# kkahatapitiya/Coarse-Fine-Networks

Measured on AMD Instinct MI355X. Metric: clips/sec (fwd+bwd+SGD) x3d_fine X3D-M T=256x224x224, higher is better.
Workload: dtype f32; 1 GPU; x3d_fine X3D-M train step (fwd+loss+bwd+SGD), 8x3x256x224x224 clips per GPU, random-init weights; clips_per_gpu=8, frames=256, parallelism=dp1, launch=eager

## Files before the change

coarse-fine-networks_amd/cfn_hip/ops.py:

```python
import torch
from torch.autograd import Function
from torch.autograd.function import once_differentiable

import ctypes
import os
import threading

from . import call, call_try, check, query, last_error, ACT_NONE, ACT_RELU, ACT_SWISH, ACT_SIGMOID


_scratch_epoch = [0]


class _ZeroArena(object):
    CHUNK = 1 << 20

    def __init__(self):
        self.buf, self.off, self.epoch = {}, {}, _scratch_epoch[0]

    def take(self, numel, dev):
        if self.epoch != _scratch_epoch[0]:
            self.buf, self.off, self.epoch = {}, {}, _scratch_epoch[0]
        numel_al = (numel + 1) & ~1
        key = (dev.type, dev.index)
# ... 440 lines not shown
        if want_w:
            g64, fin = _gw_buffers(ctx.wparam, C, 5, x.device)
        fused = want_x and want_w and call_try('cfn_dwconv_t5_bwd_fused' + _sfx(y), gy, y, gs, gq, w2, x, gx, g64, N, C, T, H * W)
        if not fused:
            if want_x:
                call('cfn_dwconv_t5_bwd_data' + _sfx(y), gy, y, gs, gq, w2, gx, N, C, T, H * W)
            if want_w:
                call('cfn_dwconv_t5_bwd_weight' + _sfx(y), gy, y, gs, gq, x, g64, N, C, T, H * W)
        if want_w:
            gw = fin()
        return gx, gw, None, None


def dwconv_t5(x, w, stats=True, out_dtype=None):
    return _DwConvT5.apply(x, w, stats, out_dtype)


class _StemConv(Function):

    @staticmethod
    def forward(ctx, x, w):
        x = check(x).contiguous()
        N, Ci, T, H, W = x.shape
        Co = w.shape[0]
        Ho, Wo = (H + 2 - 3) // 2 + 1, (W + 2 - 3) // 2 + 1
        y = torch.empty(N, Co, T, Ho, Wo, dtype=torch.float32, device=x.device)
        w2 = w.reshape(Co, Ci * 9).contiguous()
        call('cfn_stem_conv_fwd', x, w2, y, N, Ci, Co, T, H, W)
        ctx.save_for_backward(x)
        ctx.wshape = tuple(w.shape)
        ctx.wparam = w
        return y

    @staticmethod
    @once_differentiable
    def backward(ctx, gy):
        (x,) = ctx.saved_tensors
        N, Ci, T, H, W = x.shape
        Co = ctx.wshape[0]
        gw = None
        if ctx.needs_input_grad[1]:
            g64, fin = _gw_buffers(ctx.wparam, Co, Ci * 9, x.device)
            call('cfn_stem_conv_bwd_weight', gy.contiguous(), x, g64, N, Ci, Co, T, H, W)
            gw = fin()
        return None, gw


def stem_conv(x, w):
    return _StemConv.apply(x, w)


def _stem_pair_switch():
    try:
        return int(os.environ.get('CFN_STEM_PAIR', '3'))
    except ValueError:
        raise RuntimeError('CFN_STEM_PAIR must be an integer (bit 0: forward, bit 1: backward), got %r' % os.environ['CFN_STEM_PAIR'])


class _StemPair(Function):

    @staticmethod
    def forward(ctx, x, w_s, w_t, want_stats, run_frames):
        x = check(x).contiguous()
        if x.dtype != torch.float32:
            raise RuntimeError('stem_pair: fp32 clip expected, got %s' % x.dtype)
        N, Ci, T, H, W = x.shape
        Co = w_s.shape[0]
        Ho, Wo = (H + 2 - 3) // 2 + 1, (W + 2 - 3) // 2 + 1
        xs = torch.empty(N, Co, T, Ho, Wo, dtype=torch.float32, device=x.device)
        y = torch.empty_like(xs)
        s = q = None
        if want_stats:
            s, q = _f64(N, Co, x.device), _f64(N, Co, x.device)
        ws2 = w_s.reshape(Co, Ci * 9).contiguous()
        wt2 = w_t.reshape(Co, 5).contiguous()
        if not (_stem_pair_switch() & 1 and call_try('cfn_stem_pair_fwd', x, ws2, wt2, xs, y, s, q, N, Ci, Co, T, H, W, run_frames)):
            call('cfn_stem_conv_fwd', x, ws2, xs, N, Ci, Co, T, H, W)
            call('cfn_dwconv_t5_fwd', xs, wt2, y, s, q, N, Co, T, Ho * Wo)
        ctx.save_for_backward(x, xs, y, wt2)
        ctx.params = (w_s, w_t)
        ctx.run_frames = run_frames
        if not want_stats:
            return y, None, None
        return y, s, q

    @staticmethod
    @once_differentiable
    def backward(ctx, gy, gs, gq):
        x, xs, y, wt2 = ctx.saved_tensors
        w_s, w_t = ctx.params
        N, Ci, T, H, W = x.shape
        _, Co, _, Ho, Wo = xs.shape
        gy = torch.zeros_like(y) if gy is None else gy.contiguous()
        gs, gq = _opt(gs), _opt(gq)
        want_s, want_t = ctx.needs_input_grad[1], ctx.needs_input_grad[2]
        gws = gwt = None
        if want_s and want_t:
            gs64, fin_s = _gw_buffers(w_s, Co, Ci * 9, x.device)
            gt64, fin_t = _gw_buffers(w_t, Co, 5, x.device)
            if not (_stem_pair_switch() & 2 and
                    call_try('cfn_stem_pair_bwd', gy, y, gs, gq, wt2, xs, x, gt64, gs64, N, Ci, Co, T, H, W, ctx.run_frames)):
                gxs = torch.empty_like(xs)
                if not call_try('cfn_dwconv_t5_bwd_fused', gy, y, gs, gq, wt2, xs, gxs, gt64, N, Co, T, Ho * Wo):
                    call('cfn_dwconv_t5_bwd_data', gy, y, gs, gq, wt2, gxs, N, Co, T, Ho * Wo)
                    call('cfn_dwconv_t5_bwd_weight', gy, y, gs, gq, xs, gt64, N, Co, T, Ho * Wo)
                call('cfn_stem_conv_bwd_weight', gxs, x, gs64, N, Ci, Co, T, H, W)
            gws, gwt = fin_s(), fin_t()
        elif want_t:
            gt64, fin_t = _gw_buffers(w_t, Co, 5, x.device)
            call('cfn_dwconv_t5_bwd_weight', gy, y, gs, gq, xs, gt64, N, Co, T, Ho * Wo)
            gwt = fin_t()
        elif want_s:
            gs64, fin_s = _gw_buffers(w_s, Co, Ci * 9, x.device)
            gxs = torch.empty_like(xs)
            call('cfn_dwconv_t5_bwd_data', gy, y, gs, gq, wt2, gxs, N, Co, T, Ho * Wo)
            call('cfn_stem_conv_bwd_weight', gxs, x, gs64, N, Ci, Co, T, H, W)
            gws = fin_s()
        return None, gws, gwt, None, None


def stem_pair(x, w_s, w_t, stats=True, run_frames=0):
    return _StemPair.apply(x, w_s, w_t, stats, run_frames)


from .u8clips import clip_lut


def _u8_args(frames, lengths, lut):
    if frames.dtype != torch.uint8 or frames.dim() != 5 or frames.shape[4] != 3:
        raise RuntimeError('uint8 frames of shape (N, T, H, W, 3) expected, got %s %s' % (frames.dtype, tuple(frames.shape)))
    if lut.dtype != torch.float32 or lut.numel() != 3 * 256:
        raise RuntimeError('a (3, 256) fp32 table expected (ops.clip_lut), got %s %s' % (lut.dtype, tuple(lut.shape)))
    if lengths is not None:
        if lengths.numel() != frames.shape[0]:
            raise RuntimeError('one length per clip expected: %d clips, lengths %s' % (frames.shape[0], tuple(lengths.shape)))
        lengths = lengths.to(torch.int32).contiguous()
    return frames.contiguous(), lengths, lut.contiguous()


def clip_u8_to_f32(frames, lut, lengths=None):
    frames, lengths, lut = _u8_args(frames, lengths, lut)
    N, T, H, W, _ = frames.shape
    x = torch.empty(N, 3, T, H, W, dtype=torch.float32, device=frames.device)
    call('cfn_clip_u8_to_f32', frames, lut, lengths, x, N, T, H, W)
    return x


class _StemConvU8(Function):

    @staticmethod
    def forward(ctx, frames, lengths, lut, w):
        frames, lengths, lut = _u8_args(frames, lengths, lut)
        N, T, H, W, Ci = frames.shape
        Co = w.shape[0]
        Ho, Wo = (H + 2 - 3) // 2 + 1, (W + 2 - 3) // 2 + 1
        y = torch.empty(N, Co, T, Ho, Wo, dtype=torch.float32, device=frames.device)
        w2 = w.reshape(Co, Ci * 9).contiguous()
        if not call_try('cfn_stem_conv_u8_fwd', frames, lut, lengths, w2, y, N, Ci, Co, T, H, W):
            call('cfn_stem_conv_fwd', clip_u8_to_f32(frames, lut, lengths), w2, y, N, Ci, Co, T, H, W)
        ctx.save_for_backward(frames, lengths, lut)
        ctx.wshape = tuple(w.shape)
        ctx.wparam = w
        return y

    @staticmethod
    @once_differentiable
    def backward(ctx, gy):
# ... 1374 lines not shown
```

coarse-fine-networks_amd/csrc/stempair.hip:

```cpp
#include "cfn_common.h"
#include <stdlib.h>

typedef float __attribute__((ext_vector_type(16))) sp16;
typedef float __attribute__((ext_vector_type(4))) sp4;
typedef float __attribute__((ext_vector_type(2))) sp2;

struct StemPairBwdArgs {
    const float* gy; const float* y; const double* gs; const double* gq; const float* wt; const float* xs; const float* x;
    double* gwt; double* gws;
    int N, T, R, nch, runs, per_block;
};

namespace {
constexpr int SP_WI = 224, SP_WO = 112, SP_RB = 2, SP_RIN = 2 * SP_RB + 1, SP_PITCH = 228;
constexpr int SP_CIS = SP_RIN * SP_PITCH + 24;
constexpr int SP_GP = 2 * SP_WO + 2;
constexpr int SP_P = SP_WI * SP_WI, SP_PO = SP_WO * SP_WO, SP_BANDS = SP_WO / SP_RB, SP_OOB = 0x7fff0000;
constexpr int SP_XU = 3 * SP_RIN * (SP_WI / 4), SP_NXU = (SP_XU + 511) / 512;
constexpr int SP_GU = 24 * SP_RB * (SP_WO / 4), SP_NGU = (SP_GU + 511) / 512;
constexpr int SP_UPC = SP_RB * (SP_WO / 4);

struct SpCur {
    int run, n, band, ta, tb, t;
    __device__ __forceinline__ void start(int r, int R, int nch, int T) {
        run = r;
        band = r % SP_BANDS;
        const int q = r / SP_BANDS, chunk = q % nch;
        n = q / nch;
        ta = chunk * R;
        tb = min(ta + R, T);
        t = ta - 4;
    }
    __device__ __forceinline__ void next(int R, int nch, int T) {
        if (++t == tb) start(run + 1, R, nch, T);
    }
};
}

__device__ __forceinline__ float sp_taps(float a0, float a1, float a2, float a3, float a4, float w0, float w1, float w2, float w3, float w4) {
    return __builtin_fmaf(a4, w4, __builtin_fmaf(a3, w3, __builtin_fmaf(a2, w2, __builtin_fmaf(a0, w0, __fmul_rn(a1, w1)))));
}

template <bool HASY>
__global__ __launch_bounds__(512) void stem_pair_bwd_kernel(const StemPairBwdArgs a) {
    __shared__ __attribute__((aligned(16))) float lds[3 * SP_CIS + 24 * SP_GP];
    float* const img = lds;
    float* const gbuf = lds + 3 * SP_CIS;
    const int tid = threadIdx.x, lane = tid & 63, wave = cfn_uni(tid >> 6), h = lane >> 5, p = lane & 31;
    const int T = a.T, R = a.R, nch = a.nch;

    for (int i = tid; i < 3 * SP_CIS; i += 512) img[i] = 0.0f;

    int xo[SP_NXU], xl[SP_NXU], xr[SP_NXU];
#pragma unroll
    for (int k = 0; k < SP_NXU; ++k) {
        const int e = k * 512 + tid;
        const int rowid = e / (SP_WI / 4), c4 = e - rowid * (SP_WI / 4), ci = rowid / SP_RIN, r = rowid - ci * SP_RIN;
        const bool in = e < SP_XU;
        xo[k] = in ? (int)(((long)ci * T * SP_P + (long)r * SP_WI + c4 * 4) * 4) : SP_OOB;
        xl[k] = in ? ci * SP_CIS + r * SP_PITCH + 4 + c4 * 4 : -1;
        xr[k] = r;
    }
    int go[SP_NGU], gl[SP_NGU], gc[SP_NGU];
    float wk[SP_NGU][5];
#pragma unroll
    for (int k = 0; k < SP_NGU; ++k) {
        const int e = k * 512 + tid;
        const int co = e / SP_UPC, rem = e - co * SP_UPC;
        const bool in = e < SP_GU;
        go[k] = in ? (int)(((long)co * T * SP_PO + rem * 4) * 4) : SP_OOB;
        gl[k] = in ? co * SP_GP + rem * 4 : -1;
        gc[k] = in ? co : 0;
#pragma unroll
        for (int j = 0; j < 5; ++j) wk[k][j] = a.wt[gc[k] * 5 + 4 - j];
    }
    const int ohl = wave >> 2, ow0 = (wave & 3) * 28;
    const int colp = p < 27 ? p : 0;
    const int ci = colp / 9, kh = (colp - ci * 9) / 3, kw = colp - ci * 9 - kh * 3;
    const float* bp = img + ci * SP_CIS + (2 * ohl + kh) * SP_PITCH + 2 * ow0 + kw + 3 + 2 * h;
    const float* ap = gbuf + min(p, 23) * SP_GP + ohl * SP_WO + ow0 + h;

    sp16 acc0, acc1;
#pragma unroll
    for (int r = 0; r < 16; ++r) acc0[r] = acc1[r] = 0.0f;
    float acct[SP_NGU][5];
#pragma unroll
    for (int k = 0; k < SP_NGU; ++k)
#pragma unroll
        for (int j = 0; j < 5; ++j) acct[k][j] = 0.0f;

    const int first = (int)cfn_xcd_remap(blockIdx.x, gridDim.x) * a.per_block, last = min(first + a.per_block, a.runs);
    const unsigned gbytes = (unsigned)((long)24 * T * SP_PO * 4), xbytes = (unsigned)((long)3 * T * SP_P * 4);
    sp4 fg[SP_NGU], fy[SP_NGU], fs[SP_NGU], fx[SP_NXU];
    auto fetch = [&](const SpCur& c) {
        const bool on = c.run < last;
        const int n = on ? c.n : 0, f = c.t + 2;
        const bool fv = on && f >= 0 && f < T, xv = on && c.t >= c.ta;
        __amdgpu_buffer_rsrc_t rg = cfn_rsrc(a.gy + (long)n * 24 * T * SP_PO, gbytes);
        __amdgpu_buffer_rsrc_t ry = cfn_rsrc((HASY ? a.y : a.gy) + (long)n * 24 * T * SP_PO, gbytes);
        __amdgpu_buffer_rsrc_t rs = cfn_rsrc(a.xs + (long)n * 24 * T * SP_PO, gbytes);
        __amdgpu_buffer_rsrc_t rx = cfn_rsrc(a.x + (long)n * 3 * T * SP_P, xbytes);
        const int ih0 = 2 * c.band * SP_RB - 1;
        const int sg = cfn_uni(fv ? (f * SP_PO + c.band * SP_RB * SP_WO) * 4 : 0);
        const int ss = cfn_uni(xv ? (c.t * SP_PO + c.band * SP_RB * SP_WO) * 4 : 0);
        const int sx = cfn_uni(xv ? c.t * SP_P * 4 : 0), rowoff = cfn_uni(ih0 * SP_WI * 4);
#pragma unroll
        for (int k = 0; k < SP_NGU; ++k) {
            fg[k] = __builtin_bit_cast(sp4, __builtin_amdgcn_raw_buffer_load_b128(rg, fv ? go[k] : SP_OOB, sg, 0));
            if (HASY) fy[k] = __builtin_bit_cast(sp4, __builtin_amdgcn_raw_buffer_load_b128(ry, fv ? go[k] : SP_OOB, sg, 0));
        }
#pragma unroll
        for (int k = 0; k < SP_NGU; ++k)
            fs[k] = __builtin_bit_cast(sp4, __builtin_amdgcn_raw_buffer_load_b128(rs, xv ? go[k] : SP_OOB, ss, 0));
#pragma unroll
        for (int k = 0; k < SP_NXU; ++k)
            fx[k] = __builtin_bit_cast(sp4, __builtin_amdgcn_raw_buffer_load_b128(rx, (xv && xo[k] != SP_OOB && ih0 + xr[k] >= 0) ? xo[k] + rowoff : SP_OOB, sx, 0));
    };

    const sp4 zero = {0.f, 0.f, 0.f, 0.f};
    sp4 W[5][SP_NGU];
#pragma unroll
    for (int i = 0; i < 5; ++i)
#pragma unroll
        for (int k = 0; k < SP_NGU; ++k) W[i][k] = zero;
    float gsv[SP_NGU], gqv[SP_NGU];
#pragma unroll
    for (int k = 0; k < SP_NGU; ++k) gsv[k] = gqv[k] = 0.0f;

    SpCur cc, fc;
    cc.start(first, R, nch, T);
    fc = cc;
    __syncthreads();
    fetch(fc);
    fc.next(R, nch, T);
    while (cc.run < last) {
        if (cc.t == cc.ta - 4) {
#pragma unroll
            for (int k = 0; k < SP_NGU; ++k) {
                gsv[k] = a.gs ? (float)a.gs[cc.n * 24 + gc[k]] : 0.0f;
                gqv[k] = (HASY && a.gq) ? 2.0f * (float)a.gq[cc.n * 24 + gc[k]] : 0.0f;
            }
        }
        const bool mm = cc.t >= cc.ta;
        const float m = (cc.t + 2 >= 0 && cc.t + 2 < T) ? 1.0f : 0.0f;
#pragma unroll
        for (int k = 0; k < SP_NGU; ++k) {
            sp4 v = fg[k] + gsv[k];
            if (HASY) v = __builtin_elementwise_fma(fy[k], (sp4){gqv[k], gqv[k], gqv[k], gqv[k]}, v);
            W[4][k] = v * m;
        }
        if (mm) {
#pragma unroll
            for (int k = 0; k < SP_NGU; ++k) {
                sp4 gx;
#pragma unroll
                for (int i = 0; i < 4; ++i)
                    gx[i] = sp_taps(W[0][k][i], W[1][k][i], W[2][k][i], W[3][k][i], W[4][k][i], wk[k][0], wk[k][1], wk[k][2], wk[k][3], wk[k][4]);
                if (gl[k] >= 0) {
                    *reinterpret_cast<sp2*>(gbuf + gl[k]) = (sp2){gx.x, gx.y};
                    *reinterpret_cast<sp2*>(gbuf + gl[k] + 2) = (sp2){gx.z, gx.w};
                }
#pragma unroll
                for (int j = 0; j < 5; ++j) {
                    const sp4 pr = fs[k] * W[4 - j][k];
                    acct[k][j] += (pr.x + pr.y) + (pr.z + pr.w);
                }
            }
#pragma unroll
            for (int k = 0; k < SP_NXU; ++k)
                if (xl[k] >= 0) *reinterpret_cast<sp4*>(img + xl[k]) = fx[k];
            __syncthreads();
        }
        fetch(fc);
        fc.next(R, nch, T);
        if (mm) {
#pragma unroll
            for (int j = 0; j < 14; j += 2) {
                acc0 = __builtin_amdgcn_mfma_f32_32x32x2f32(ap[2 * j], bp[4 * j], acc0, 0, 0, 0);
                acc1 = __builtin_amdgcn_mfma_f32_32x32x2f32(ap[2 * j + 2], bp[4 * j + 4], acc1, 0, 0, 0);
            }
            __syncthreads();
        }
#pragma unroll
        for (int i = 0; i < 4; ++i)
#pragma unroll
            for (int k = 0; k < SP_NGU; ++k) W[i][k] = W[i + 1][k];
        cc.next(R, nch, T);
    }

    __syncthreads();
#pragma unroll
    for (int k = 0; k < SP_NGU; ++k)
        if (gl[k] >= 0) {
#pragma unroll
            for (int j = 0; j < 5; ++j) lds[(k * 512 + tid) * 5 + j] = acct[k][j];
        }
    __syncthreads();
    if (tid < 24 * 5) {
        const int co = tid / 5, j = tid - co * 5;
        float s = 0.0f;
        for (int u = 0; u < SP_UPC; ++u) s += lds[(co * SP_UPC + u) * 5 + j];
        cfn_add64(&a.gwt[co * 5 + j], (double)s);
    }
    __syncthreads();
#pragma unroll
    for (int r = 0; r < 16; ++r) lds[(wave * 16 + r) * 64 + lane] = acc0[r] + acc1[r];
    __syncthreads();
    for (int e = tid; e < 16 * 64; e += 512) {
        const int r = e >> 6, l = e & 63, hh = l >> 5, col = l & 31;
        const int co = (r & 3) + 8 * (r >> 2) + 4 * hh;
        float s = 0.0f;
#pragma unroll
        for (int w = 0; w < 8; ++w) s += lds[(w * 16 + r) * 64 + l];
        if (co < 24 && col < 27) cfn_add64(&a.gws[co * 27 + col], (double)s);
    }
}

static int stem_pair_plan(int N, int T, int wgs) {
    int best = T;
    long best_cost = -1;
    for (int nch = 1; nch == 1 || T / nch >= 32; ++nch) {
        const int R = cfn_cdiv(T, nch);
        const long runs = (long)N * cfn_cdiv(T, R) * SP_BANDS, per = (runs + wgs - 1) / wgs, cost = per * (R + 2);
        if (best_cost < 0 || cost < best_cost) { best_cost = cost; best = R; }
    }
    return best;
}

static int stem_pair_cus() {
    static int cus = 0;
    if (!cus) { int dev = 0; hipDeviceProp_t pr; cus = (hipGetDevice(&dev) == hipSuccess && hipGetDeviceProperties(&pr, dev) == hipSuccess) ? pr.multiProcessorCount : 256; }
    return cus;
}

static bool stem_pair_shape_ok(int Cimg, int Cout, int T, int Hi, int Wi) {
    return Cimg == 3 && Cout == 24 && Hi == SP_WI && Wi == SP_WI && (long)24 * T * SP_PO * 4 < 0x7fff0000L;
}

extern "C" int cfn_stem_pair_bwd(const float* gy, const float* y, const double* gsum, const double* gsumsq, const float* w_t, const float* xs,
                                 const float* x, double* gw_t, double* gw_s, int N, int Cimg, int Cout, int T, int Hi, int Wi, int run_frames,
                                 void* stream) {
    CFN_REQUIRE(gy && w_t && xs && x && gw_t && gw_s, "cfn_stem_pair_bwd: null tensor");
    CFN_REQUIRE(gsumsq == nullptr || y != nullptr, "cfn_stem_pair_bwd: gsumsq needs y");
    CFN_REQUIRE(N > 0 && Cimg > 0 && Cout > 0 && T > 0 && Hi > 0 && Wi > 0 && run_frames >= 0, "cfn_stem_pair_bwd: bad shape");
    if (!stem_pair_shape_ok(Cimg, Cout, T, Hi, Wi)) return -1;
    const bool hasy = y != nullptr && gsumsq != nullptr;
    if ((((uintptr_t)gy | (uintptr_t)xs | (uintptr_t)x | (uintptr_t)(hasy ? y : gy)) & 15) != 0) return -1;
    const int wgs = stem_pair_cus();
    const int R = run_frames > 0 ? (run_frames < T ? run_frames : T) : stem_pair_plan(N, T, wgs);
    const int nch = cfn_cdiv(T, R);
    const long runs = (long)N * nch * SP_BANDS;
    if (runs >= (1L << 30)) return -1;
    long blocks = runs < wgs ? runs : wgs;
    const long per = (runs + blocks - 1) / blocks;
    blocks = (runs + per - 1) / per;
    StemPairBwdArgs a = {gy, hasy ? y : nullptr, gsum, hasy ? gsumsq : nullptr, w_t, xs, x, gw_t, gw_s, N, T, R, nch, (int)runs, (int)per};
    hipStream_t st = (hipStream_t)stream;
    CfnProfScope prof(CFN_K_STEM, st, 4.0 * N * T * ((double)3 * SP_P + (double)24 * SP_PO * (hasy ? 3 : 2)));
    if (hasy) hipLaunchKernelGGL(stem_pair_bwd_kernel<true>, dim3((unsigned)blocks), dim3(512), 0, st, a);
    else hipLaunchKernelGGL(stem_pair_bwd_kernel<false>, dim3((unsigned)blocks), dim3(512), 0, st, a);
    return cfn_check_launch("stem_pair_bwd");
}

static constexpr __host__ __device__ int sp_tap(int k) { return k < 27 ? (k / 9) * SP_CIS + ((k % 9) / 3) * SP_PITCH + k % 3 : 0; }

struct StemPairFwdArgs {
    const float* x; const float* ws; const float* wt; float* xs; float* y; double* s1; double* s2;
    int N, T, R, nch, runs;
};

__global__ __launch_bounds__(448, 4) void stem_pair_fwd_kernel(const StemPairFwdArgs a) {
    constexpr int NT = 448, NXU = (SP_XU + NT - 1) / NT, KP = 14;
    __shared__ __attribute__((aligned(16))) float img[2][3 * SP_CIS];
    __shared__ __attribute__((aligned(16))) float wts[24 * 8];
    __shared__ float wsl[14 * 64];
    __shared__ float red[2][7][24];
    const int tid = threadIdx.x, lane = tid & 63, wave = cfn_uni(tid >> 6), half = lane >> 5, col = lane & 31;
    const int T = a.T;
    SpCur c;
    c.start((int)cfn_xcd_remap(blockIdx.x, gridDim.x), a.R, a.nch, T);
    const int n = c.n, band = c.band, ta = c.ta, tb = c.tb;

    for (int i = tid; i < 2 * 3 * SP_CIS; i += NT) (&img[0][0])[i] = 0.0f;
    if (tid < 24 * 5) wts[(tid / 5) * 8 + tid % 5] = a.wt[tid];

    const int ih0 = 2 * band * SP_RB - 1;
    int xo[NXU], xl[NXU];
#pragma unroll
    for (int k = 0; k < NXU; ++k) {
        const int e = k * NT + tid;
        const int rowid = e / (SP_WI / 4), c4 = e - rowid * (SP_WI / 4), ci = rowid / SP_RIN, r = rowid - ci * SP_RIN;
        const bool in = e < SP_XU;
        xo[k] = (in && ih0 + r >= 0) ? (int)(((long)ci * T * SP_P + (long)(ih0 + r) * SP_WI + c4 * 4) * 4) : SP_OOB;
        xl[k] = in ? ci * SP_CIS + r * SP_PITCH + 4 + c4 * 4 : -1;
    }
    if (wave == 0) {
#pragma unroll
        for (int s = 0; s < KP; ++s) {
            const int k = 2 * s + half;
            wsl[s * 64 + lane] = (k < 27 && col < 24) ? a.ws[col * 27 + k] : 0.0f;
        }
    }
    const int pos = wave * 32 + col, ohl = pos / SP_WO, ow = pos - ohl * SP_WO;
    const int lboff = 2 * ohl * SP_PITCH + 2 * ow + 3;

    const unsigned gbytes = (unsigned)((long)24 * T * SP_PO * 4), xbytes = (unsigned)((long)3 * T * SP_P * 4);
    __amdgpu_buffer_rsrc_t rx = cfn_rsrc(a.x + (long)n * 3 * T * SP_P, xbytes);
    __amdgpu_buffer_rsrc_t rs = cfn_rsrc(a.xs + (long)n * 24 * T * SP_PO, gbytes);
    __amdgpu_buffer_rsrc_t ry = cfn_rsrc(a.y + (long)n * 24 * T * SP_PO, gbytes);
    const int vout = (half * 4 * T * SP_PO + band * SP_RB * SP_WO + pos) * 4;

    sp4 fx[NXU];
    auto fetch = [&](int s) {
        const bool fv = s >= 0 && s < T && s <= tb + 1;
        const int sx = cfn_uni(fv ? s * SP_P * 4 : 0);
#pragma unroll
        for (int k = 0; k < NXU; ++k)
            fx[k] = __builtin_bit_cast(sp4, __builtin_amdgcn_raw_buffer_load_b128(rx, fv ? xo[k] : SP_OOB, sx, 0));
    };
    auto put = [&](int b) {
#pragma unroll
        for (int k = 0; k < NXU; ++k)
            if (xl[k] >= 0) *reinterpret_cast<sp4*>(&img[b][xl[k]]) = fx[k];
    };

    float W[5][12], st1[12], st2[12];
#pragma unroll
    for (int r = 0; r < 12; ++r) {
        st1[r] = st2[r] = 0.0f;
#pragma unroll
        for (int i = 0; i < 5; ++i) W[i][r] = 0.0f;
    }

    fetch(ta - 2);
    __syncthreads();
    put(0);
    fetch(ta - 1);
    __syncthreads();
    int b = 0;
    for (int s = ta - 2; s <= tb + 1; ++s, b ^= 1) {
        put(b ^ 1);
        fetch(s + 2);
        const float* lb = &img[b][lboff];
        int hsel = half;
        asm volatile("" : "+v"(hsel));
        sp16 acc;
#pragma unroll
        for (int r = 0; r < 16; ++r) acc[r] = 0.0f;
#pragma unroll
        for (int k = 0; k < KP; ++k) acc = __builtin_amdgcn_mfma_f32_32x32x2f32(wsl[k * 64 + lane], lb[hsel ? sp_tap(2 * k + 1) : sp_tap(2 * k)], acc, 0, 0, 0);
        const bool own = s >= ta && s < tb, emit = s - 2 >= ta;
#pragma unroll
        for (int r = 0; r < 12; ++r) {
            const int cr = (r & 3) + 8 * (r >> 2);
            W[4][r] = acc[r];
            __builtin_amdgcn_raw_buffer_store_b32(__builtin_bit_cast(unsigned, W[4][r]), rs, own ? vout : SP_OOB, cfn_uni(own ? (cr * T + s) * SP_PO * 4 : 0), 0);
        }
        if (emit) {
#pragma unroll
            for (int r = 0; r < 12; ++r) {
                const int cr = (r & 3) + 8 * (r >> 2);
                const float* wk = wts + (cr + 4 * half) * 8;
                const float yv = sp_taps(W[0][r], W[1][r], W[2][r], W[3][r], W[4][r], wk[0], wk[1], wk[2], wk[3], wk[4]);
                __builtin_amdgcn_raw_buffer_store_b32(__builtin_bit_cast(unsigned, yv), ry, vout, cfn_uni((cr * T + s - 2) * SP_PO * 4), 0);
                st1[r] += yv;
                st2[r] += yv * yv;
            }
        }
#pragma unroll
        for (int i = 0; i < 4; ++i)
#pragma unroll
            for (int r = 0; r < 12; ++r) W[i][r] = W[i + 1][r];
        __syncthreads();
    }
    if (a.s1) {
#pragma unroll
        for (int r = 0; r < 12; ++r) {
#pragma unroll
            for (int o = 16; o > 0; o >>= 1) { st1[r] += __shfl_xor(st1[r], o, 64); st2[r] += __shfl_xor(st2[r], o, 64); }
            if (col == 0) {
                const int co = (r & 3) + 8 * (r >> 2) + 4 * half;
                red[0][wave][co] = st1[r];
                red[1][wave][co] = st2[r];
            }
        }
        __syncthreads();
        if (tid < 48) {
            const int which = tid / 24, co = tid - which * 24;
            float v = 0.0f;
#pragma unroll
            for (int w = 0; w < 7; ++w) v += red[which][w][co];
            cfn_add64((which ? a.s2 : a.s1) + n * 24 + co, (double)v);
        }
    }
}

static int stem_pair_fwd_plan(int N, int T, int slots) {
    int best = T;
    long best_cost = -1;
    for (int nch = 1; nch == 1 || T / nch >= 32; ++nch) {
        const int R = cfn_cdiv(T, nch);
        const long runs = (long)N * cfn_cdiv(T, R) * SP_BANDS, rounds = (runs + slots - 1) / slots, cost = rounds * (R + 4);
        if (best_cost < 0 || cost < best_cost) { best_cost = cost; best = R; }
    }
    return best;
}

extern "C" int cfn_stem_pair_fwd(const float* x, const float* w_s, const float* w_t, float* xs, float* y, double* sum, double* sumsq, int N,
                                 int Cimg, int Cout, int T, int Hi, int Wi, int run_frames, void* stream) {
    CFN_REQUIRE(x && w_s && w_t && xs && y, "cfn_stem_pair_fwd: null tensor");
    CFN_REQUIRE((sum == nullptr) == (sumsq == nullptr), "cfn_stem_pair_fwd: sum/sumsq mismatch");
    CFN_REQUIRE(N > 0 && Cimg > 0 && Cout > 0 && T > 0 && Hi > 0 && Wi > 0 && run_frames >= 0, "cfn_stem_pair_fwd: bad shape");
    if (!stem_pair_shape_ok(Cimg, Cout, T, Hi, Wi)) return -1;
    if ((((uintptr_t)x | (uintptr_t)xs | (uintptr_t)y) & 15) != 0) return -1;
    const int R = run_frames > 0 ? (run_frames < T ? run_frames : T) : stem_pair_fwd_plan(N, T, 2 * stem_pair_cus());
    const int nch = cfn_cdiv(T, R);
    const long runs = (long)N * nch * SP_BANDS;
    if (runs >= (1L << 30)) return -1;
    StemPairFwdArgs a = {x, w_s, w_t, xs, y, sum, sumsq, N, T, R, nch, (int)runs};
    hipStream_t st = (hipStream_t)stream;
    CfnProfScope prof(CFN_K_STEM, st, 4.0 * N * T * ((double)3 * SP_P + (double)24 * SP_PO * 2));
    hipLaunchKernelGGL(stem_pair_fwd_kernel, dim3((unsigned)runs), dim3(448), 0, st, a);
    return cfn_check_launch("stem_pair_fwd");
}
```

include/cfn_hip.h:

```cpp
#ifndef CFN_HIP_H
#define CFN_HIP_H
#ifdef __cplusplus
extern "C" {
#endif

const char* cfn_last_error(void);
const char* cfn_version(void);
int cfn_device_info(int* cus, int* lds_per_cu, char* name, int name_len);

int cfn_prof_enable(int family, int on);
int cfn_prof_collect(int family, double* total_ms, long* launches, double* total_bytes);

int cfn_dwconv3d_fwd(const float* x, const double* A, const double* B, int act, const float* w, float* y, double* sum,
                     double* sumsq, int N, int C, int T, int Hi, int Wi, int stride, void* stream);
int cfn_dwconv3d_bwd_data(const float* gy, const float* y, const double* gsum, const double* gsumsq, const float* w,
                          const float* x, const double* A, const double* B, int act, float* gx, double* gA, double* gB,
                          int N, int C, int T, int Hi, int Wi, int stride, void* stream);
int cfn_dwconv3d_bwd_weight(const float* gy, const float* y, const double* gsum, const double* gsumsq, const float* x,
                            const double* A, const double* B, int act, double* gw, int N, int C, int T, int Hi, int Wi,
                            int stride, void* stream);
int cfn_dwconv3d_bwd_fused(const float* gy, const float* y, const double* gsum, const double* gsumsq, const float* w,
                           const float* x, const double* A, const double* B, int act, float* gx, double* gA, double* gB,
                           double* gw, int N, int C, int T, int H, int W, void* stream);
int cfn_dwconv3d_bwd_fused_s2(const float* gy, const float* y, const double* gsum, const double* gsumsq, const float* w,
                              const float* x, const double* A, const double* B, int act, float* gx, double* gA, double* gB,
                              double* gw, int N, int C, int T, int H, int W, void* stream);

int cfn_dwconv_t5_fwd(const float* x, const float* w, float* y, double* sum, double* sumsq, int N, int C, int T,
                      long plane, void* stream);
int cfn_dwconv_t5_bwd_data(const float* gy, const float* y, const double* gsum, const double* gsumsq, const float* w,
                           float* gx, int N, int C, int T, long plane, void* stream);
int cfn_dwconv_t5_bwd_weight(const float* gy, const float* y, const double* gsum, const double* gsumsq, const float* x,
                             double* gw, int N, int C, int T, long plane, void* stream);
int cfn_dwconv_t5_bwd_fused(const float* gy, const float* y, const double* gsum, const double* gsumsq, const float* w,
                            const float* x, float* gx, double* gw, int N, int C, int T, long plane, void* stream);

int cfn_pwconv_fwd(const float* x, const double* A, const double* B, int act, const float* w, float* y, double* sum,
                   double* sumsq, int N, int Cin, int Cout, int T, int Hi, int Wi, int stride, void* stream);
int cfn_pwconv_bwd_data(const float* gy, const float* y, const double* gsum, const double* gsumsq, const float* w,
                        const float* x, const double* A, const double* B, int act, float* gx, double* gA, double* gB, int N,
                        int Cin, int Cout, int T, int Hi, int Wi, int stride, void* stream);
int cfn_pwconv_bwd_data_acc(const float* gy, const float* y, const double* gsum, const double* gsumsq, const float* w,
                        const float* x, const double* A, const double* B, int act, float* gx, double* gA, double* gB, int N,
                        int Cin, int Cout, int T, int Hi, int Wi, int stride, const float* acc, int acc_stride,
                        const double* gscale, void* stream);
int cfn_pwconv_bwd_weight(const float* gy, const float* y, const double* gsum, const double* gsumsq, const float* x,
                          const double* A, const double* B, int act, double* gw, int N, int Cin, int Cout, int T, int Hi,
                          int Wi, int stride, const double* gscale, void* stream);

int cfn_pw_split_terms(int terms);

int cfn_pwconv_route(int op, int N, int Cin, int Cout, int T, int Hi, int Wi, int stride, int act, int flags, char* out, int cap);

int cfn_deterministic(int on);

int cfn_pwconv_bwd_fused(const float* gy, const float* y, const double* gsum, const double* gsumsq, const float* w,
                         const float* x, const double* A, const double* B, int act, float* gx, double* gA, double* gB,
                         double* gw, int N, int Cin, int Cout, int T, int Hi, int Wi, const float* acc, int acc_stride,
                         const double* gscale, void* stream);

int cfn_pwconv_short_bwd(const float* gy, const float* y, const double* gsum, const double* gsumsq, const double* gscale,
                         const float* w, const float* x, const double* A, const double* B, int act, float* da, double* gw,
                         int N, int Cin, int Cout, int T, int Hi, int Wi, int stride, void* stream);

int cfn_stem_conv_fwd(const float* x, const float* w, float* y, int N, int Cimg, int Cout, int T, int Hi, int Wi,
                      void* stream);
int cfn_stem_conv_bwd_weight(const float* gy, const float* x, double* gw, int N, int Cimg, int Cout, int T, int Hi, int Wi,
                             void* stream);

int cfn_stem_pair_fwd(const float* x, const float* w_s, const float* w_t, float* xs, float* y, double* sum, double* sumsq, int N,
                      int Cimg, int Cout, int T, int Hi, int Wi, int run_frames, void* stream);
int cfn_stem_pair_bwd(const float* gy, const float* y, const double* gsum, const double* gsumsq, const float* w_t, const float* xs,
                      const float* x, double* gw_t, double* gw_s, int N, int Cimg, int Cout, int T, int Hi, int Wi, int run_frames,
                      void* stream);

int cfn_clip_u8_to_f32(const unsigned char* frames, const float* lut, const int* lengths, float* x, int N, int T, int H, int W,
                       void* stream);
int cfn_stem_conv_u8_fwd(const unsigned char* frames, const float* lut, const int* lengths, const float* w, float* y, int N,
                         int Cimg, int Cout, int T, int Hi, int Wi, void* stream);
int cfn_stem_conv_u8_bwd_weight(const float* gy, const unsigned char* frames, const float* lut, const int* lengths, double* gw,
                                int N, int Cimg, int Cout, int T, int Hi, int Wi, void* stream);

int cfn_bn_fold_fwd(const double* s, const double* q, const float* gamma, const float* beta, float* run_mean, float* run_var,
                    long* nbt, int training, int N, int C, int S, double count, double eps, double momentum, const float* w1,
                    const float* b1, const float* w2, const float* b2, int Wd, double pool_count, double* A, double* B,
                    double* mean, double* rstd, float* A0, float* B0, float* gate, float* hbuf, float* pooled, void* stream);
int cfn_bn_fold_bwd(const double* gA, const double* gB, const double* s, const float* gamma, const double* mean,
                    const double* rstd, const float* A0, const float* B0, const float* gate, const float* hbuf,
                    const float* pooled, const float* w1, const float* w2, int training, int N, int C, int S, int Wd,
                    double count, double pool_count, double* gs, double* gq, float* ggamma, float* gbeta, float* gw1,
                    float* gb1, float* gw2, float* gb2, double* tA, double* tB, void* stream);

int cfn_conv3d_dense_fwd(const float* x, const double* A, const double* B, int act, const float* w, float* y, double* sum,
                         double* sumsq, int N, int Cin, int Cout, int T, int Hi, int Wi, const int* geom, void* stream);
int cfn_conv3d_dense_bwd_data(const float* gy, const float* y, const double* gsum, const double* gsumsq, const float* w,
                              const float* x, const double* A, const double* B, int act, float* gx, double* gA, double* gB,
                              int N, int Cin, int Cout, int T, int Hi, int Wi, const int* geom, void* stream);
int cfn_conv3d_dense_bwd_weight(const float* gy, const float* y, const double* gsum, const double* gsumsq, const float* x,
                                const double* A, const double* B, int act, double* gw, int N, int Cin, int Cout, int T, int Hi,
                                int Wi, const int* geom, void* stream);
int cfn_conv3d_dense_route(int op, int N, int Cin, int Cout, int T, int Hi, int Wi, const int* geom, int flags, int cus, char* out, int cap);

int cfn_gauss_align_fwd(const long* meta, const float* mask, const float* gx, double tx, double ratio, float* GX, int B, int crops,
                        int Tf, int K, void* stream);
int cfn_gauss_align_bwd(const float* gGX, const long* meta, const float* mask, const float* gx, double tx, double ratio,
                        float* ggx, int B, int crops, int Tf, int K, void* stream);

int cfn_fusion_gather_fwd(const float* x, const float* at_raw, const float* at_bias, const float* GX, const float* mask, float* z,
                          float* den, int B, int crops, int C, int Tf, int K, int P, void* stream);
int cfn_fusion_gather_bwd(const float* gz, const float* z, const float* den, const float* x, const float* at_raw,
                          const float* at_bias, const float* GX, const float* mask, float* gx, float* gat, float* gGX, float* dw,
                          int B, int crops, int C, int Tf, int K, int P, void* stream);

int cfn_bn_add_relu_fwd(const float* y, const double* A, const double* B, const float* res, const double* Ar, const double* Br,
                        float* out, int* mask, long NC, long vol, void* stream);
int cfn_bn_add_relu_bwd(const float* gout, const float* gout2, const float* out, const float* y, const double* A, const float* res,
                        const double* Ar, float* gy, float* gres, double* gA, double* gB, double* gAr, long NC, long vol,
                        void* stream);
long cfn_bn_add_relu_mask_words(long NC, long vol);
int cfn_bn_add_relu_bwd_g(const float* gout, const float* gout2, const float* out, const int* mask, const float* y,
                          const float* res, float* g, double* gA, double* gB, double* gAr, long NC, long vol, void* stream);

int cfn_affine_act_fwd(const float* x, const double* A, const double* B, int act, float* out, long NC, long vol, void* stream);
int cfn_affine_act_bwd(const float* gout, const float* x, const double* A, const double* B, int act, float* gx, double* gA,
                       double* gB, long NC, long vol, void* stream);
int cfn_channel_stats(const float* x, double* sum, double* sumsq, long NC, long vol, void* stream);

// ... 222 lines not shown
```

Measured before the change: 107.7 clips/s.

## Recompute stem conv output in backward instead of storing intermediate xs

The forward stem pair kernel gains a variant that skips writing the intermediate spatial conv output xs. The backward kernel gains an RC variant that recomputes xs per tile in LDS from the already-staged input image using MFMA with the spatial weights, then uses it for the temporal weight gradient. This removes a full activation-sized write in forward and a read in backward, and saves memory. The cost is extra MFMA work and LDS in the backward kernel, which could lower occupancy.

After: 108.3 clips/s (median of 6 runs). No clear change (+0.6%).

```diff
diff --git a/coarse-fine-networks_amd/cfn_hip/ops.py b/coarse-fine-networks_amd/cfn_hip/ops.py
--- a/coarse-fine-networks_amd/cfn_hip/ops.py
+++ b/coarse-fine-networks_amd/cfn_hip/ops.py
@@ -516,9 +516,15 @@
 
 def _stem_pair_switch():
     try:
-        return int(os.environ.get('CFN_STEM_PAIR', '3'))
+        return int(os.environ.get('CFN_STEM_PAIR', '7'))
     except ValueError:
-        raise RuntimeError('CFN_STEM_PAIR must be an integer (bit 0: forward, bit 1: backward), got %r' % os.environ['CFN_STEM_PAIR'])
+        raise RuntimeError('CFN_STEM_PAIR must be an integer (bit 0: forward, bit 1: backward, bit 2: do not keep xs), got %r'
+                           % os.environ['CFN_STEM_PAIR'])
+
+
+def _stem_pair_rc_accepts(x, y, Ci, Co, run_frames):
+    N, _, T, H, W = x.shape
+    return query('cfn_stem_pair_bwd_rc_accepts', y.data_ptr(), y.data_ptr(), x.data_ptr(), N, Ci, Co, T, H, W, run_frames) == 1
 
 
 class _StemPair(Function):
@@ -531,17 +537,25 @@
         N, Ci, T, H, W = x.shape
         Co = w_s.shape[0]
         Ho, Wo = (H + 2 - 3) // 2 + 1, (W + 2 - 3) // 2 + 1
-        xs = torch.empty(N, Co, T, Ho, Wo, dtype=torch.float32, device=x.device)
-        y = torch.empty_like(xs)
+        y = torch.empty(N, Co, T, Ho, Wo, dtype=torch.float32, device=x.device)
         s = q = None
         if want_stats:
             s, q = _f64(N, Co, x.device), _f64(N, Co, x.device)
         ws2 = w_s.reshape(Co, Ci * 9).contiguous()
         wt2 = w_t.reshape(Co, 5).contiguous()
-        if not (_stem_pair_switch() & 1 and call_try('cfn_stem_pair_fwd', x, ws2, wt2, xs, y, s, q, N, Ci, Co, T, H, W, run_frames)):
-            call('cfn_stem_conv_fwd', x, ws2, xs, N, Ci, Co, T, H, W)
-            call('cfn_dwconv_t5_fwd', xs, wt2, y, s, q, N, Co, T, Ho * Wo)
-        ctx.save_for_backward(x, xs, y, wt2)
+        sw = _stem_pair_switch()
+        xs = None
+        if not ((sw & 7) == 7 and _stem_pair_rc_accepts(x, y, Ci, Co, run_frames)
+                and call_try('cfn_stem_pair_fwd', x, ws2, wt2, None, y, s, q, N, Ci, Co, T, H, W, run_frames)):
+            xs = torch.empty_like(y)
+            if not (sw & 1 and call_try('cfn_stem_pair_fwd', x, ws2, wt2, xs, y, s, q, N, Ci, Co, T, H, W, run_frames)):
+                call('cfn_stem_conv_fwd', x, ws2, xs, N, Ci, Co, T, H, W)
+                call('cfn_dwconv_t5_fwd', xs, wt2, y, s, q, N, Co, T, Ho * Wo)
+        if xs is None:
+            ctx.save_for_backward(x, y, wt2, ws2)
+        else:
+            ctx.save_for_backward(x, y, wt2, xs)
+        ctx.kept_xs = xs is not None
         ctx.params = (w_s, w_t)
         ctx.run_frames = run_frames
         if not want_stats:
@@ -551,32 +565,44 @@
     @staticmethod
     @once_differentiable
     def backward(ctx, gy, gs, gq):
-        x, xs, y, wt2 = ctx.saved_tensors
+        x, y, wt2, last = ctx.saved_tensors
         w_s, w_t = ctx.params
         N, Ci, T, H, W = x.shape
-        _, Co, _, Ho, Wo = xs.shape
+        _, Co, _, Ho, Wo = y.shape
         gy = torch.zeros_like(y) if gy is None else gy.contiguous()
         gs, gq = _opt(gs), _opt(gq)
         want_s, want_t = ctx.needs_input_grad[1], ctx.needs_input_grad[2]
         gws = gwt = None
+        kept = ctx.kept_xs
+
+        def stored_xs():
+            if kept:
+                return last
+            xs = torch.empty_like(y)
+            call('cfn_stem_conv_fwd', x, last, xs, N, Ci, Co, T, H, W)
+            return xs
+
         if want_s and want_t:
             gs64, fin_s = _gw_buffers(w_s, Co, Ci * 9, x.device)
             gt64, fin_t = _gw_buffers(w_t, Co, 5, x.device)
-            if not (_stem_pair_switch() & 2 and
-                    call_try('cfn_stem_pair_bwd', gy, y, gs, gq, wt2, xs, x, gt64, gs64, N, Ci, Co, T, H, W, ctx.run_frames)):
-                gxs = torch.empty_like(xs)
-                if not call_try('cfn_dwconv_t5_bwd_fused', gy, y, gs, gq, wt2, xs, gxs, gt64, N, Co, T, Ho * Wo):
-                    call('cfn_dwconv_t5_bwd_data', gy, y, gs, gq, wt2, gxs, N, Co, T, Ho * Wo)
-                    call('cfn_dwconv_t5_bwd_weight', gy, y, gs, gq, xs, gt64, N, Co, T, Ho * Wo)
-                call('cfn_stem_conv_bwd_weight', gxs, x, gs64, N, Ci, Co, T, H, W)
+            sw = _stem_pair_switch()
+            if not ((sw & 6) == 6 and not kept and
+                    call_try('cfn_stem_pair_bwd_rc', gy, y, gs, gq, wt2, last, x, gt64, gs64, N, Ci, Co, T, H, W, ctx.run_frames)):
+                xs = stored_xs()
+                if not (sw & 2 and call_try('cfn_stem_pair_bwd', gy, y, gs, gq, wt2, xs, x, gt64, gs64, N, Ci, Co, T, H, W, ctx.run_frames)):
+                    gxs = torch.empty_like(xs)
+                    if not call_try('cfn_dwconv_t5_bwd_fused', gy, y, gs, gq, wt2, xs, gxs, gt64, N, Co, T, Ho * Wo):
+                        call('cfn_dwconv_t5_bwd_data', gy, y, gs, gq, wt2, gxs, N, Co, T, Ho * Wo)
+                        call('cfn_dwconv_t5_bwd_weight', gy, y, gs, gq, xs, gt64, N, Co, T, Ho * Wo)
+                    call('cfn_stem_conv_bwd_weight', gxs, x, gs64, N, Ci, Co, T, H, W)
             gws, gwt = fin_s(), fin_t()
         elif want_t:
             gt64, fin_t = _gw_buffers(w_t, Co, 5, x.device)
-            call('cfn_dwconv_t5_bwd_weight', gy, y, gs, gq, xs, gt64, N, Co, T, Ho * Wo)
+            call('cfn_dwconv_t5_bwd_weight', gy, y, gs, gq, stored_xs(), gt64, N, Co, T, Ho * Wo)
             gwt = fin_t()
         elif want_s:
             gs64, fin_s = _gw_buffers(w_s, Co, Ci * 9, x.device)
-            gxs = torch.empty_like(xs)
+            gxs = torch.empty_like(y)
             call('cfn_dwconv_t5_bwd_data', gy, y, gs, gq, wt2, gxs, N, Co, T, Ho * Wo)
             call('cfn_stem_conv_bwd_weight', gxs, x, gs64, N, Ci, Co, T, H, W)
             gws = fin_s()
diff --git a/coarse-fine-networks_amd/csrc/stempair.hip b/coarse-fine-networks_amd/csrc/stempair.hip
--- a/coarse-fine-networks_amd/csrc/stempair.hip
+++ b/coarse-fine-networks_amd/csrc/stempair.hip
@@ -7,6 +7,7 @@
 
 struct StemPairBwdArgs {
     const float* gy; const float* y; const double* gs; const double* gq; const float* wt; const float* xs; const float* x;
+    const float* ws;
     double* gwt; double* gws;
     int N, T, R, nch, runs, per_block;
 };
@@ -41,15 +42,25 @@
     return __builtin_fmaf(a4, w4, __builtin_fmaf(a3, w3, __builtin_fmaf(a2, w2, __builtin_fmaf(a0, w0, __fmul_rn(a1, w1)))));
 }
 
-template <bool HASY>
+static constexpr __host__ __device__ int sp_tap(int k) { return k < 27 ? (k / 9) * SP_CIS + ((k % 9) / 3) * SP_PITCH + k % 3 : 0; }
+
+template <bool HASY, bool RC>
 __global__ __launch_bounds__(512) void stem_pair_bwd_kernel(const StemPairBwdArgs a) {
-    __shared__ __attribute__((aligned(16))) float lds[3 * SP_CIS + 24 * SP_GP];
+    __shared__ __attribute__((aligned(16))) float lds[3 * SP_CIS + 24 * SP_GP + (RC ? 24 * SP_GP + 14 * 64 : 0)];
     float* const img = lds;
     float* const gbuf = lds + 3 * SP_CIS;
+    float* const xsb = gbuf + 24 * SP_GP;
+    float* const wsl = xsb + 24 * SP_GP;
     const int tid = threadIdx.x, lane = tid & 63, wave = cfn_uni(tid >> 6), h = lane >> 5, p = lane & 31;
     const int T = a.T, R = a.R, nch = a.nch;
 
     for (int i = tid; i < 3 * SP_CIS; i += 512) img[i] = 0.0f;
+    if constexpr (RC) {
+        for (int i = tid; i < 14 * 64; i += 512) {
+            const int k = 2 * (i >> 6) + ((i & 63) >> 5), co = i & 31;
+            wsl[i] = (k < 27 && co < 24) ? a.ws[co * 27 + k] : 0.0f;
+        }
+    }
 
     int xo[SP_NXU], xl[SP_NXU], xr[SP_NXU];
 #pragma unroll
@@ -79,6 +90,9 @@
     const int ci = colp / 9, kh = (colp - ci * 9) / 3, kw = colp - ci * 9 - kh * 3;
     const float* bp = img + ci * SP_CIS + (2 * ohl + kh) * SP_PITCH + 2 * ow0 + kw + 3 + 2 * h;
     const float* ap = gbuf + min(p, 23) * SP_GP + ohl * SP_WO + ow0 + h;
+    const float* xb = img + 2 * ohl * SP_PITCH + 2 * (ow0 + min(p, 27)) + 3;
+    float* const xw = xsb + 4 * h * SP_GP + ohl * SP_WO + ow0 + p;
+    const float* const xb1 = xb + h, * const xb2 = xb + h * (SP_PITCH - 2);
 
     sp16 acc0, acc1;
 #pragma unroll
@@ -98,7 +112,7 @@
         const bool fv = on && f >= 0 && f < T, xv = on && c.t >= c.ta;
         __amdgpu_buffer_rsrc_t rg = cfn_rsrc(a.gy + (long)n * 24 * T * SP_PO, gbytes);
         __amdgpu_buffer_rsrc_t ry = cfn_rsrc((HASY ? a.y : a.gy) + (long)n * 24 * T * SP_PO, gbytes);
-        __amdgpu_buffer_rsrc_t rs = cfn_rsrc(a.xs + (long)n * 24 * T * SP_PO, gbytes);
+        __amdgpu_buffer_rsrc_t rs = cfn_rsrc((RC ? a.gy : a.xs) + (long)n * 24 * T * SP_PO, gbytes);
         __amdgpu_buffer_rsrc_t rx = cfn_rsrc(a.x + (long)n * 3 * T * SP_P, xbytes);
         const int ih0 = 2 * c.band * SP_RB - 1;
         const int sg = cfn_uni(fv ? (f * SP_PO + c.band * SP_RB * SP_WO) * 4 : 0);
@@ -109,9 +123,11 @@
             fg[k] = __builtin_bit_cast(sp4, __builtin_amdgcn_raw_buffer_load_b128(rg, fv ? go[k] : SP_OOB, sg, 0));
             if (HASY) fy[k] = __builtin_bit_cast(sp4, __builtin_amdgcn_raw_buffer_load_b128(ry, fv ? go[k] : SP_OOB, sg, 0));
         }
-#pragma unroll
-        for (int k = 0; k < SP_NGU; ++k)
-            fs[k] = __builtin_bit_cast(sp4, __builtin_amdgcn_raw_buffer_load_b128(rs, xv ? go[k] : SP_OOB, ss, 0));
+        if constexpr (!RC) {
+#pragma unroll
+            for (int k = 0; k < SP_NGU; ++k)
+                fs[k] = __builtin_bit_cast(sp4, __builtin_amdgcn_raw_buffer_load_b128(rs, xv ? go[k] : SP_OOB, ss, 0));
+        }
 #pragma unroll
         for (int k = 0; k < SP_NXU; ++k)
             fx[k] = __builtin_bit_cast(sp4, __builtin_amdgcn_raw_buffer_load_b128(rx, (xv && xo[k] != SP_OOB && ih0 + xr[k] >= 0) ? xo[k] + rowoff : SP_OOB, sx, 0));
@@ -160,10 +176,12 @@
                     *reinterpret_cast<sp2*>(gbuf + gl[k]) = (sp2){gx.x, gx.y};
                     *reinterpret_cast<sp2*>(gbuf + gl[k] + 2) = (sp2){gx.z, gx.w};
                 }
-#pragma unroll
-                for (int j = 0; j < 5; ++j) {
-                    const sp4 pr = fs[k] * W[4 - j][k];
-                    acct[k][j] += (pr.x + pr.y) + (pr.z + pr.w);
+                if constexpr (!RC) {
+#pragma unroll
+                    for (int j = 0; j < 5; ++j) {
+                        const sp4 pr = fs[k] * W[4 - j][k];
+                        acct[k][j] += (pr.x + pr.y) + (pr.z + pr.w);
+                    }
                 }
             }
 #pragma unroll
@@ -174,12 +192,41 @@
         fetch(fc);
         fc.next(R, nch, T);
         if (mm) {
+            if constexpr (RC) {
+                int hsel = h;
+                asm volatile("" : "+v"(hsel));
+                sp16 xa;
+#pragma unroll
+                for (int r = 0; r < 16; ++r) xa[r] = 0.0f;
+#pragma unroll
+                for (int k = 0; k < 14; ++k) {
+                    const int d = sp_tap(2 * k + 1) - sp_tap(2 * k);
+                    const float bv = d == 1 ? xb1[sp_tap(2 * k)] : d == SP_PITCH - 2 ? xb2[sp_tap(2 * k)] : xb[hsel ? sp_tap(2 * k + 1) : sp_tap(2 * k)];
+                    xa = __builtin_amdgcn_mfma_f32_32x32x2f32(wsl[k * 64 + lane], bv, xa, 0, 0, 0);
+                }
+                if (p < 28) {
+#pragma unroll
+                    for (int r = 0; r < 12; ++r) xw[((r & 3) + 8 * (r >> 2)) * SP_GP] = xa[r];
+                }
+            }
 #pragma unroll
             for (int j = 0; j < 14; j += 2) {
                 acc0 = __builtin_amdgcn_mfma_f32_32x32x2f32(ap[2 * j], bp[4 * j], acc0, 0, 0, 0);
                 acc1 = __builtin_amdgcn_mfma_f32_32x32x2f32(ap[2 * j + 2], bp[4 * j + 4], acc1, 0, 0, 0);
             }
             __syncthreads();
+            if constexpr (RC) {
+#pragma unroll
+                for (int k = 0; k < SP_NGU; ++k) {
+                    const float* const xp = xsb + max(gl[k], 0);
+                    const sp2 lo = *reinterpret_cast<const sp2*>(xp), hi = *reinterpret_cast<const sp2*>(xp + 2);
+#pragma unroll
+                    for (int j = 0; j < 5; ++j) {
+                        const sp2 pl = lo * (sp2){W[4 - j][k].x, W[4 - j][k].y}, ph = hi * (sp2){W[4 - j][k].z, W[4 - j][k].w};
+                        acct[k][j] += (pl.x + pl.y) + (ph.x + ph.y);
+                    }
+                }
+            }
         }
 #pragma unroll
         for (int i = 0; i < 4; ++i)
@@ -237,38 +284,72 @@
     return Cimg == 3 && Cout == 24 && Hi == SP_WI && Wi == SP_WI && (long)24 * T * SP_PO * 4 < 0x7fff0000L;
 }
 
+static bool stem_pair_bwd_accepts(const float* gy, const float* y, const float* xs, const float* x, int N, int Cimg, int Cout, int T, int Hi, int Wi,
+                                  int run_frames, int* R_out) {
+    if (N <= 0 || T <= 0 || run_frames < 0 || !stem_pair_shape_ok(Cimg, Cout, T, Hi, Wi)) return false;
+    if ((((uintptr_t)gy | (uintptr_t)xs | (uintptr_t)x | (uintptr_t)y) & 15) != 0) return false;
+    const int R = run_frames > 0 ? (run_frames < T ? run_frames : T) : stem_pair_plan(N, T, stem_pair_cus());
+    if ((long)N * cfn_cdiv(T, R) * SP_BANDS >= (1L << 30)) return false;
+    if (R_out) *R_out = R;
+    return true;
+}
+
+static int stem_pair_bwd_launch(const char* what, const float* gy, const float* y, const double* gsum, const double* gsumsq, const float* w_t,
+                                const float* xs, const float* w_s, const float* x, double* gw_t, double* gw_s, int N, int Cimg, int Cout, int T,
+                                int Hi, int Wi, int run_frames, void* stream) {
+    const bool hasy = y != nullptr && gsumsq != nullptr, rc = xs == nullptr;
+    int R = 0;
+    if (!stem_pair_bwd_accepts(gy, hasy ? y : gy, xs, x, N, Cimg, Cout, T, Hi, Wi, run_frames, &R)) return -1;
+    const int wgs = stem_pair_cus();
+    const int nch = cfn_cdiv(T, R);
+    const long runs = (long)N * nch * SP_BANDS;
+    long blocks = runs < wgs ? runs : wgs;
+    const long per = (runs + blocks - 1) / blocks;
+    blocks = (runs + per - 1) / per;
+    StemPairBwdArgs a = {gy, hasy ? y : nullptr, gsum, hasy ? gsumsq : nullptr, w_t, xs, x, w_s, gw_t, gw_s, N, T, R, nch, (int)runs, (int)per};
+    hipStream_t st = (hipStream_t)stream;
+    CfnProfScope prof(CFN_K_STEM, st, 4.0 * N * T * ((double)3 * SP_P + (double)24 * SP_PO * ((hasy ? 3 : 2) - (rc ? 1 : 0))));
+    const dim3 grid((unsigned)blocks), block(512);
+    if (rc) {
+        if (hasy) hipLaunchKernelGGL((stem_pair_bwd_kernel<true, true>), grid, block, 0, st, a);
+        else hipLaunchKernelGGL((stem_pair_bwd_kernel<false, true>), grid, block, 0, st, a);
+    } else {
+        if (hasy) hipLaunchKernelGGL((stem_pair_bwd_kernel<true, false>), grid, block, 0, st, a);
+        else hipLaunchKernelGGL((stem_pair_bwd_kernel<false, false>), grid, block, 0, st, a);
+    }
+    return cfn_check_launch(what);
+}
+
 extern "C" int cfn_stem_pair_bwd(const float* gy, const float* y, const double* gsum, const double* gsumsq, const float* w_t, const float* xs,
                                  const float* x, double* gw_t, double* gw_s, int N, int Cimg, int Cout, int T, int Hi, int Wi, int run_frames,
                                  void* stream) {
     CFN_REQUIRE(gy && w_t && xs && x && gw_t && gw_s, "cfn_stem_pair_bwd: null tensor");
     CFN_REQUIRE(gsumsq == nullptr || y != nullptr, "cfn_stem_pair_bwd: gsumsq needs y");
     CFN_REQUIRE(N > 0 && Cimg > 0 && Cout > 0 && T > 0 && Hi > 0 && Wi > 0 && run_frames >= 0, "cfn_stem_pair_bwd: bad shape");
-    if (!stem_pair_shape_ok(Cimg, Cout, T, Hi, Wi)) return -1;
-    const bool hasy = y != nullptr && gsumsq != nullptr;
-    if ((((uintptr_t)gy | (uintptr_t)xs | (uintptr_t)x | (uintptr_t)(hasy ? y : gy)) & 15) != 0) return -1;
-    const int wgs = stem_pair_cus();
-    const int R = run_frames > 0 ? (run_frames < T ? run_frames : T) : stem_pair_plan(N, T, wgs);
-    const int nch = cfn_cdiv(T, R);
-    const long runs = (long)N * nch * SP_BANDS;
-    if (runs >= (1L << 30)) return -1;
-    long blocks = runs < wgs ? runs : wgs;
-    const long per = (runs + blocks - 1) / blocks;
-    blocks = (runs + per - 1) / per;
-    StemPairBwdArgs a = {gy, hasy ? y : nullptr, gsum, hasy ? gsumsq : nullptr, w_t, xs, x, gw_t, gw_s, N, T, R, nch, (int)runs, (int)per};
-    hipStream_t st = (hipStream_t)stream;
-    CfnProfScope prof(CFN_K_STEM, st, 4.0 * N * T * ((double)3 * SP_P + (double)24 * SP_PO * (hasy ? 3 : 2)));
-    if (hasy) hipLaunchKernelGGL(stem_pair_bwd_kernel<true>, dim3((unsigned)blocks), dim3(512), 0, st, a);
-    else hipLaunchKernelGGL(stem_pair_bwd_kernel<false>, dim3((unsigned)blocks), dim3(512), 0, st, a);
-    return cfn_check_launch("stem_pair_bwd");
-}
-
-static constexpr __host__ __device__ int sp_tap(int k) { return k < 27 ? (k / 9) * SP_CIS + ((k % 9) / 3) * SP_PITCH + k % 3 : 0; }
+    return stem_pair_bwd_launch("stem_pair_bwd", gy, y, gsum, gsumsq, w_t, xs, nullptr, x, gw_t, gw_s, N, Cimg, Cout, T, Hi, Wi, run_frames, stream);
+}
+
+extern "C" int cfn_stem_pair_bwd_rc(const float* gy, const float* y, const double* gsum, const double* gsumsq, const float* w_t, const float* w_s,
+                                    const float* x, double* gw_t, double* gw_s, int N, int Cimg, int Cout, int T, int Hi, int Wi, int run_frames,
+                                    void* stream) {
+    CFN_REQUIRE(gy && w_t && w_s && x && gw_t && gw_s, "cfn_stem_pair_bwd_rc: null tensor");
+    CFN_REQUIRE(gsumsq == nullptr || y != nullptr, "cfn_stem_pair_bwd_rc: gsumsq needs y");
+    CFN_REQUIRE(N > 0 && Cimg > 0 && Cout > 0 && T > 0 && Hi > 0 && Wi > 0 && run_frames >= 0, "cfn_stem_pair_bwd_rc: bad shape");
+    return stem_pair_bwd_launch("stem_pair_bwd_rc", gy, y, gsum, gsumsq, w_t, nullptr, w_s, x, gw_t, gw_s, N, Cimg, Cout, T, Hi, Wi, run_frames, stream);
+}
+
+extern "C" int cfn_stem_pair_bwd_rc_accepts(const float* gy, const float* y, const float* x, int N, int Cimg, int Cout, int T, int Hi, int Wi,
+                                            int run_frames) {
+    return stem_pair_bwd_accepts(gy, y ? y : gy, nullptr, x, N, Cimg, Cout, T, Hi, Wi, run_frames, nullptr) ? 1 : 0;
+}
+
 
 struct StemPairFwdArgs {
     const float* x; const float* ws; const float* wt; float* xs; float* y; double* s1; double* s2;
     int N, T, R, nch, runs;
 };
 
+template <bool STORE>
 __global__ __launch_bounds__(448, 4) void stem_pair_fwd_kernel(const StemPairFwdArgs a) {
     constexpr int NT = 448, NXU = (SP_XU + NT - 1) / NT, KP = 14;
     __shared__ __attribute__((aligned(16))) float img[2][3 * SP_CIS];
@@ -306,7 +387,7 @@
 
     const unsigned gbytes = (unsigned)((long)24 * T * SP_PO * 4), xbytes = (unsigned)((long)3 * T * SP_P * 4);
     __amdgpu_buffer_rsrc_t rx = cfn_rsrc(a.x + (long)n * 3 * T * SP_P, xbytes);
-    __amdgpu_buffer_rsrc_t rs = cfn_rsrc(a.xs + (long)n * 24 * T * SP_PO, gbytes);
+    __amdgpu_buffer_rsrc_t rs = cfn_rsrc((STORE ? a.xs : a.y) + (long)n * 24 * T * SP_PO, gbytes);
     __amdgpu_buffer_rsrc_t ry = cfn_rsrc(a.y + (long)n * 24 * T * SP_PO, gbytes);
     const int vout = (half * 4 * T * SP_PO + band * SP_RB * SP_WO + pos) * 4;
 
@@ -354,7 +435,7 @@
         for (int r = 0; r < 12; ++r) {
             const int cr = (r & 3) + 8 * (r >> 2);
             W[4][r] = acc[r];
-            __builtin_amdgcn_raw_buffer_store_b32(__builtin_bit_cast(unsigned, W[4][r]), rs, own ? vout : SP_OOB, cfn_uni(own ? (cr * T + s) * SP_PO * 4 : 0), 0);
+            if constexpr (STORE) __builtin_amdgcn_raw_buffer_store_b32(__builtin_bit_cast(unsigned, W[4][r]), rs, own ? vout : SP_OOB, cfn_uni(own ? (cr * T + s) * SP_PO * 4 : 0), 0);
         }
         if (emit) {
 #pragma unroll
@@ -408,7 +489,7 @@
 
 extern "C" int cfn_stem_pair_fwd(const float* x, const float* w_s, const float* w_t, float* xs, float* y, double* sum, double* sumsq, int N,
                                  int Cimg, int Cout, int T, int Hi, int Wi, int run_frames, void* stream) {
-    CFN_REQUIRE(x && w_s && w_t && xs && y, "cfn_stem_pair_fwd: null tensor");
+    CFN_REQUIRE(x && w_s && w_t && y, "cfn_stem_pair_fwd: null tensor");
     CFN_REQUIRE((sum == nullptr) == (sumsq == nullptr), "cfn_stem_pair_fwd: sum/sumsq mismatch");
     CFN_REQUIRE(N > 0 && Cimg > 0 && Cout > 0 && T > 0 && Hi > 0 && Wi > 0 && run_frames >= 0, "cfn_stem_pair_fwd: bad shape");
     if (!stem_pair_shape_ok(Cimg, Cout, T, Hi, Wi)) return -1;
@@ -419,7 +500,8 @@
     if (runs >= (1L << 30)) return -1;
     StemPairFwdArgs a = {x, w_s, w_t, xs, y, sum, sumsq, N, T, R, nch, (int)runs};
     hipStream_t st = (hipStream_t)stream;
-    CfnProfScope prof(CFN_K_STEM, st, 4.0 * N * T * ((double)3 * SP_P + (double)24 * SP_PO * 2));
-    hipLaunchKernelGGL(stem_pair_fwd_kernel, dim3((unsigned)runs), dim3(448), 0, st, a);
+    CfnProfScope prof(CFN_K_STEM, st, 4.0 * N * T * ((double)3 * SP_P + (double)24 * SP_PO * (xs ? 2 : 1)));
+    if (xs) hipLaunchKernelGGL(stem_pair_fwd_kernel<true>, dim3((unsigned)runs), dim3(448), 0, st, a);
+    else hipLaunchKernelGGL(stem_pair_fwd_kernel<false>, dim3((unsigned)runs), dim3(448), 0, st, a);
     return cfn_check_launch("stem_pair_fwd");
 }
diff --git a/include/cfn_hip.h b/include/cfn_hip.h
--- a/include/cfn_hip.h
+++ b/include/cfn_hip.h
@@ -73,6 +73,11 @@
 int cfn_stem_pair_bwd(const float* gy, const float* y, const double* gsum, const double* gsumsq, const float* w_t, const float* xs,
                       const float* x, double* gw_t, double* gw_s, int N, int Cimg, int Cout, int T, int Hi, int Wi, int run_frames,
                       void* stream);
+int cfn_stem_pair_bwd_rc(const float* gy, const float* y, const double* gsum, const double* gsumsq, const float* w_t, const float* w_s,
+                         const float* x, double* gw_t, double* gw_s, int N, int Cimg, int Cout, int T, int Hi, int Wi, int run_frames,
+                         void* stream);
+int cfn_stem_pair_bwd_rc_accepts(const float* gy, const float* y, const float* x, int N, int Cimg, int Cout, int T, int Hi, int Wi,
+                                 int run_frames);
 
 int cfn_clip_u8_to_f32(const unsigned char* frames, const float* lut, const int* lengths, float* x, int N, int T, int H, int W,
                        void* stream);
```
